# GabeTsai/YOLO-For-Turbines

Measured on AMD Instinct MI355X. Metric: images/sec at 416x416 (fwd), higher is better.
Workload: dtype f32; 1 GPU; BASELINE configs[1]: batch 32/GPU 416x416 fp32 inference, 80-class head, YOLOv3 forward (75 fused conv launches); per_gpu_batch=32, global_batch=32, image_size=416, num_classes=80, parallelism=image-sharded x1 (no collective)

## Files before the change

yolo_for_turbines_amd/csrc/conv_f32_epilogue.h:

```cpp
#pragma once
#include "common.h"

namespace yolo {

typedef float f32x16 __attribute__((ext_vector_type(16)));

struct ConvArgs {
    const float* x;
    const float* w;
    const char* w_planes;
    const float* scale;
    const float* shift;
    const float* res;
    float* y;
    int* nan_flag;
    int N, H, W, Cin, Cout, Ho, Wo, M;
    int ks, stride, pad;
    int x_ld, x_off, y_ld, y_off, r_ld, r_off;
    int Kpad, KT;
    int act, out_mode, flags;
    int nc5;
    int tiles_n;
};

constexpr int BK = 32;

int conv_igemm_launch(const ConvArgs& a, int tile, hipStream_t s);

bool split3_supported(const yolo_conv_desc* d);
bool split3_eligible(const yolo_conv_desc* d);
int conv_split3_launch(const ConvArgs& a, int tile, hipStream_t s);
size_t split3_weight_bytes(const yolo_conv_desc* d);
int split3_weights_launch(const yolo_conv_desc* d, const void* w_packed, void* out, hipStream_t s);

bool splitk_supported(const yolo_conv_desc* d);
bool splitk_eligible(const yolo_conv_desc* d);
int splitk_slices(const yolo_conv_desc* d, int* steps);
size_t splitk_workspace_bytes(const yolo_conv_desc* d);
int conv_splitk_launch(const ConvArgs& a, const yolo_conv_desc* d, void* ws, size_t ws_bytes, hipStream_t s);

__device__ __forceinline__ void conv_f32_store4(const ConvArgs& p, int m, int n, f32x4 v, int HoWo, bool has_res, bool nan_chk, bool& saw_nan) {
    if (has_res) v += *reinterpret_cast<const f32x4*>(p.res + (size_t)m * p.r_ld + p.r_off + n);
    if (nan_chk && (v[0] != v[0] || v[1] != v[1] || v[2] != v[2] || v[3] != v[3])) saw_nan = true;
    if (p.out_mode == YOLO_OUT_NHWC) {
        *reinterpret_cast<f32x4*>(p.y + (size_t)m * p.y_ld + p.y_off + n) = v;
    } else {
        const int img = m / HoWo;
        const int rem = m - img * HoWo;
        const int ho = rem / p.Wo;
        const int wo = rem - ho * p.Wo;
        const int W2 = 2 * p.Wo;
        float* d = p.y + ((size_t)(img * 2 * p.Ho + 2 * ho) * W2 + 2 * wo) * p.y_ld + p.y_off + n;
        *reinterpret_cast<f32x4*>(d) = v;
        *reinterpret_cast<f32x4*>(d + p.y_ld) = v;
        *reinterpret_cast<f32x4*>(d + (size_t)W2 * p.y_ld) = v;
        *reinterpret_cast<f32x4*>(d + (size_t)(W2 + 1) * p.y_ld) = v;
    }
}

__device__ __forceinline__ void conv_f32_store1(const ConvArgs& p, int m, int n, float v, int HoWo, int head_a, int head_k, bool has_res,
                                                bool nan_chk, bool& saw_nan) {
    if (has_res) v += p.res[(size_t)m * p.r_ld + p.r_off + n];
    if (nan_chk && v != v) saw_nan = true;
    if (p.out_mode == YOLO_OUT_NHWC) {
        p.y[(size_t)m * p.y_ld + p.y_off + n] = v;
    } else {
        const int img = m / HoWo;
        const int rem = m - img * HoWo;
        const int ho = rem / p.Wo;
        const int wo = rem - ho * p.Wo;
        if (p.out_mode == YOLO_OUT_UPSAMPLE2X) {
            const int W2 = 2 * p.Wo;
            float* d = p.y + ((size_t)(img * 2 * p.Ho + 2 * ho) * W2 + 2 * wo) * p.y_ld + p.y_off + n;
            d[0] = v;
            d[p.y_ld] = v;
            d[(size_t)W2 * p.y_ld] = v;
            d[(size_t)(W2 + 1) * p.y_ld] = v;
        } else {
            p.y[((size_t)((img * 3 + head_a) * p.Ho + ho) * p.Wo + wo) * p.nc5 + head_k] = v;
        }
    }
}

template <int BM, int BN>
__device__ __forceinline__ void conv_f32_epilogue(const ConvArgs& p, f32x16 (&acc)[BM / 64][BN / 64], float* ost, int m0, int n0) {
    constexpr int WM = BM / 2, WN = BN / 2;
    constexpr int TM = WM / 32, TN = WN / 32;
    const int tid = threadIdx.x;
    const int lane = tid & 63;
    const int wave = tid >> 6;
    const int wm = wave >> 1, wn = wave & 1;
    const int frow = lane & 31, fh = lane >> 5;
    const int HoWo = p.Ho * p.Wo;
    const bool has_res = p.flags & YOLO_FLAG_RESIDUAL;
    const bool nan_chk = p.flags & YOLO_FLAG_NANCHECK;
    bool saw_nan = false;
    const bool aligned4 = ((p.y_ld | p.y_off) & 3) == 0 && (!has_res || ((p.r_ld | p.r_off) & 3) == 0);
    if (p.out_mode != YOLO_OUT_HEAD && (p.Cout & 3) == 0 && aligned4) {
        constexpr int OLD = BN + 4;
#pragma unroll
        for (int j = 0; j < TN; ++j) {
            const int n = n0 + wn * WN + j * 32 + frow;
            const bool nv = n < p.Cout;
            const float sc = nv ? p.scale[n] : 0.f;
            const float sh = nv ? p.shift[n] : 0.f;
            float* dst = ost + wn * WN + j * 32 + frow;
            YOLO_SWITCH_ACT(p.act,
                _Pragma("unroll") for (int i = 0; i < TM; ++i)
                    _Pragma("unroll") for (int r = 0; r < 16; ++r) {
                        const int row = wm * WM + i * 32 + (r & 3) + 8 * (r >> 2) + 4 * fh;
                        dst[row * OLD] = act_c<ACT>(acc[i][j][r] * sc + sh);
                    })
        }
        __syncthreads();
        constexpr int C4 = BN / 4;
#pragma unroll 4
        for (int idx = tid; idx < BM * C4; idx += 256) {
            const int row = idx / C4, c4 = idx - row * C4;
            const int m = m0 + row, n = n0 + c4 * 4;
            if (m >= p.M || n >= p.Cout) continue;
            conv_f32_store4(p, m, n, *reinterpret_cast<const f32x4*>(ost + row * OLD + c4 * 4), HoWo, has_res, nan_chk, saw_nan);
        }
        if (nan_chk && saw_nan) atomicOr(p.nan_flag, 2);
        return;
    }
#pragma unroll
    for (int j = 0; j < TN; ++j) {
        const int n = n0 + wn * WN + j * 32 + frow;
        const bool nv = n < p.Cout;
        const float sc = nv ? p.scale[n] : 0.f;
        const float sh = nv ? p.shift[n] : 0.f;
        int head_a = 0, head_k = 0;
        if (p.out_mode == YOLO_OUT_HEAD) {
            head_a = n / p.nc5;
            head_k = n - head_a * p.nc5;
        }
        YOLO_SWITCH_ACT(p.act,
            _Pragma("unroll") for (int i = 0; i < TM; ++i)
                _Pragma("unroll") for (int r = 0; r < 16; ++r) acc[i][j][r] = act_c<ACT>(acc[i][j][r] * sc + sh);)
#pragma unroll
        for (int i = 0; i < TM; ++i) {
#pragma unroll
            for (int r = 0; r < 16; ++r) {
                const int m = m0 + wm * WM + i * 32 + (r & 3) + 8 * (r >> 2) + 4 * fh;
                if (m >= p.M || !nv) continue;
                conv_f32_store1(p, m, n, acc[i][j][r], HoWo, head_a, head_k, has_res, nan_chk, saw_nan);
            }
        }
    }
    if (nan_chk && saw_nan) atomicOr(p.nan_flag, 2);
}

}
```

yolo_for_turbines_amd/csrc/conv_split3_f32.hip:

```cpp
#include "conv_f32_epilogue.h"
#include "split3.h"

namespace yolo {

constexpr int S3_ROWB = 64;

__device__ __forceinline__ int s3_row_off(int r, int chunk) { return r * S3_ROWB + (((chunk >> 1) ^ ((r >> 2) & 3)) * 16 + (chunk & 1) * 8); }

typedef const __attribute__((address_space(1))) void* s3_gptr;
typedef __attribute__((address_space(3))) void* s3_lptr;
__device__ __forceinline__ void s3_glds16(const void* g, void* l) { __builtin_amdgcn_global_load_lds((s3_gptr)g, (s3_lptr)l, 16, 0, 0); }

struct S3PrepArgs {
    const float* w;
    char* out;
    int Kpad, KT, cp;
};

__global__ __launch_bounds__(256) void split3_weights_f32(const S3PrepArgs p) {
    const int tid = threadIdx.x;
    const int chunk = tid & 7;
    const int n = blockIdx.x * 32 + (tid >> 3);
    const size_t plane_b = (size_t)p.cp * S3_ROWB;
    const float* src = p.w + (size_t)n * p.Kpad + chunk * 4;
    char* dst = p.out + s3_row_off(n, chunk);
    f32x4 chk = {0.f, 0.f, 0.f, 0.f};
    for (int kt = 0; kt < p.KT; ++kt) {
        const f32x4 v = *reinterpret_cast<const f32x4*>(src + kt * BK);
        u32x2 h, m, l;
        s3_split(v, h, m, l, chk);
        char* d = dst + (size_t)kt * 3 * plane_b;
        *reinterpret_cast<u32x2*>(d) = h;
        *reinterpret_cast<u32x2*>(d + plane_b) = m;
        *reinterpret_cast<u32x2*>(d + 2 * plane_b) = l;
    }
    const bool nonfinite = chk[0] != chk[0] || chk[1] != chk[1] || chk[2] != chk[2] || chk[3] != chk[3];
    const int any = __syncthreads_or(nonfinite);
    if (tid == 0) reinterpret_cast<unsigned*>(p.out + (size_t)p.KT * 3 * plane_b)[blockIdx.x] = any ? 1u : 0u;
}

template <int BM, int BN, bool WREADY, bool WDMA>
__global__ __launch_bounds__(256, 2) void conv_split3_f32(const ConvArgs p) {
    static_assert(WREADY || !WDMA, "LDS-DMA needs the prepared weights");
    constexpr int WM = BM / 2, WN = BN / 2;
    constexpr int TM = WM / 32, TN = WN / 32;
    constexpr int RA = BM / 32, RB = BN / 32;
    constexpr bool DBUF = BM + BN <= 128;
    constexpr int A_BYTES = 3 * BM * S3_ROWB;
    constexpr int B_BYTES = 3 * BN * S3_ROWB;
    constexpr int BUF_BYTES = A_BYTES + B_BYTES;
    constexpr bool BRING = DBUF || WDMA;
    constexpr int B_SLOT = DBUF ? BUF_BYTES : B_BYTES;
    constexpr int PB = BN / 64;
    extern __shared__ __attribute__((aligned(16))) char smem_raw[];

    const int tid = threadIdx.x;
    const int lane = tid & 63;
    const int wave = tid >> 6;
    const int wm = wave >> 1, wn = wave & 1;
    const int tile_n = blockIdx.x % p.tiles_n;
    const int tile_m = blockIdx.x / p.tiles_n;
    const int m0 = tile_m * BM, n0 = tile_n * BN;
    const int HoWo = p.Ho * p.Wo;

    auto row_geom = [&](int m, long long& base, unsigned& mask) {
        const bool mv = m < p.M;
        const int mm = mv ? m : 0;
        const int n = mm / HoWo;
        const int rem = mm - n * HoWo;
        const int ho = rem / p.Wo;
        const int wo = rem - ho * p.Wo;
        const int hi0 = ho * p.stride - p.pad, wi0 = wo * p.stride - p.pad;
        base = ((long long)(n * p.H + hi0) * p.W + wi0) * p.x_ld + p.x_off;
        unsigned mk = 0;
        for (int kh = 0; kh < p.ks; ++kh)
            for (int kw = 0; kw < p.ks; ++kw)
                if (mv && (unsigned)(hi0 + kh) < (unsigned)p.H && (unsigned)(wi0 + kw) < (unsigned)p.W)
                    mk |= 1u << (kh * p.ks + kw);
        mask = mk;
    };

    const int chunk = tid & 7;
    const int lrow = tid >> 3;
    long long a_base[RA];
    unsigned a_mask[RA];
#pragma unroll
    for (int i = 0; i < RA; ++i) row_geom(m0 + lrow + 32 * i, a_base[i], a_mask[i]);
    const float* wrow = p.w + (size_t)(n0 + lrow) * p.Kpad + chunk * 4;
    const char* wq = p.w_planes;
    const size_t plane_b = (size_t)((p.Cout + 127) & ~127) * S3_ROWB;
    const char* wsrc = wq + (size_t)n0 * S3_ROWB + tid * 16;

    f32x4 ra[RA], rb[RB];
    s3_u32x4 rw[3][PB];
    f32x4 chk = {0.f, 0.f, 0.f, 0.f};
    auto load_global = [&](int kt) {
        const int kg = kt * BK;
        const int tap = kg / p.Cin;
        const int coff = kg - tap * p.Cin + chunk * 4;
        const int kh = tap / p.ks, kw = tap - kh * p.ks;
        const long long toff = (long long)(kh * p.W + kw) * p.x_ld + coff;
#pragma unroll
        for (int i = 0; i < RA; ++i) {
            const bool v = (a_mask[i] >> tap) & 1u;
            f32x4 z = {0.f, 0.f, 0.f, 0.f};
            ra[i] = v ? *reinterpret_cast<const f32x4*>(p.x + a_base[i] + toff) : z;
        }
        if constexpr (!WREADY) {
#pragma unroll
            for (int i = 0; i < RB; ++i)
                rb[i] = *reinterpret_cast<const f32x4*>(wrow + (size_t)(32 * i) * p.Kpad + kt * BK);
        } else {
            const char* src = wsrc + (size_t)kt * 3 * plane_b;
            char* dst = smem_raw + A_BYTES + (kt & 1) * B_SLOT + wave * 1024;
#pragma unroll
            for (int q = 0; q < 3; ++q)
#pragma unroll
                for (int i = 0; i < PB; ++i) {
                    if constexpr (WDMA)
                        s3_glds16(src + q * plane_b + i * 4096, dst + q * BN * S3_ROWB + i * 4096);
                    else
                        rw[q][i] = *reinterpret_cast<const s3_u32x4*>(src + q * plane_b + i * 4096);
                }
        }
    };
    auto store_lds = [&](int buf, int bslot) {
        char* a = smem_raw + buf * BUF_BYTES + s3_row_off(lrow, chunk);
        char* b = smem_raw + A_BYTES + bslot * B_SLOT + s3_row_off(lrow, chunk);
#pragma unroll
        for (int i = 0; i < RA; ++i) {
            u32x2 h, m, l;
            s3_split(ra[i], h, m, l, chk);
            *reinterpret_cast<u32x2*>(a + (0 * BM + 32 * i) * S3_ROWB) = h;
            *reinterpret_cast<u32x2*>(a + (1 * BM + 32 * i) * S3_ROWB) = m;
            *reinterpret_cast<u32x2*>(a + (2 * BM + 32 * i) * S3_ROWB) = l;
        }
        if constexpr (!WREADY) {
#pragma unroll
            for (int i = 0; i < RB; ++i) {
                u32x2 h, m, l;
                s3_split(rb[i], h, m, l, chk);
                *reinterpret_cast<u32x2*>(b + (0 * BN + 32 * i) * S3_ROWB) = h;
                *reinterpret_cast<u32x2*>(b + (1 * BN + 32 * i) * S3_ROWB) = m;
                *reinterpret_cast<u32x2*>(b + (2 * BN + 32 * i) * S3_ROWB) = l;
            }
        } else if constexpr (!WDMA) {
            char* bw = smem_raw + A_BYTES + bslot * B_SLOT + tid * 16;
#pragma unroll
            for (int q = 0; q < 3; ++q)
#pragma unroll
                for (int i = 0; i < PB; ++i) *reinterpret_cast<s3_u32x4*>(bw + q * BN * S3_ROWB + i * 4096) = rw[q][i];
        }
    };

    f32x16 acc[TM][TN];
#pragma unroll
    for (int i = 0; i < TM; ++i)
#pragma unroll
        for (int j = 0; j < TN; ++j)
#pragma unroll
            for (int r = 0; r < 16; ++r) acc[i][j][r] = 0.f;

    const int frow = lane & 31, fh = lane >> 5;
    const int a_frag = (wm * WM + frow) * S3_ROWB;
    const int b_frag = A_BYTES + (wn * WN + frow) * S3_ROWB;
    const int fsw = (frow >> 2) & 3;
    const int f_slot[2] = {(fh ^ fsw) * 16, ((2 + fh) ^ fsw) * 16};

    load_global(0);
    store_lds(0, 0);
    if constexpr (WDMA) asm volatile("s_waitcnt vmcnt(0)" ::: "memory");
    __syncthreads();

    for (int kt = 0; kt < p.KT; ++kt) {
        const int cur = DBUF ? (kt & 1) : 0;
        const int bcur = BRING ? (kt & 1) : 0;
        const bool more = kt + 1 < p.KT;
        if (more) load_global(kt + 1);
        const char* Ab = smem_raw + cur * BUF_BYTES + a_frag;
        const char* Bb = smem_raw + bcur * B_SLOT + b_frag;
#pragma unroll
        for (int c = 0; c < 2; ++c) {
            s3_bf16x8 af[TM][3], bf[TN][3];
#pragma unroll
            for (int i = 0; i < TM; ++i)
#pragma unroll
                for (int q = 0; q < 3; ++q)
                    af[i][q] = *reinterpret_cast<const s3_bf16x8*>(Ab + (q * BM + i * 32) * S3_ROWB + f_slot[c]);
#pragma unroll
            for (int j = 0; j < TN; ++j)
#pragma unroll
                for (int q = 0; q < 3; ++q)
                    bf[j][q] = *reinterpret_cast<const s3_bf16x8*>(Bb + (q * BN + j * 32) * S3_ROWB + f_slot[c]);
            constexpr int QA[6] = {0, 2, 1, 0, 1, 0};
            constexpr int QB[6] = {2, 0, 1, 1, 0, 0};
#pragma unroll
            for (int t = 0; t < 6; ++t)
#pragma unroll
                for (int i = 0; i < TM; ++i)
#pragma unroll
                    for (int j = 0; j < TN; ++j)
                        acc[i][j] = __builtin_amdgcn_mfma_f32_32x32x16_bf16(af[i][QA[t]], bf[j][QB[t]], acc[i][j], 0, 0, 0);
        }
        if (!DBUF) __syncthreads();
        if (more) store_lds(DBUF ? (cur ^ 1) : 0, BRING ? (bcur ^ 1) : 0);
        if constexpr (WDMA) asm volatile("s_waitcnt vmcnt(0)" ::: "memory");
        __syncthreads();
    }

    bool nonfinite = chk[0] != chk[0] || chk[1] != chk[1] || chk[2] != chk[2] || chk[3] != chk[3];
    if constexpr (WREADY) {
        const unsigned* table = reinterpret_cast<const unsigned*>(wq + (size_t)p.KT * 3 * plane_b);
#pragma unroll
        for (int g = 0; g < BN / 32; ++g) nonfinite |= table[n0 / 32 + g] != 0;
    }
    if (__syncthreads_or(nonfinite)) {
        long long f_base[TM];
        unsigned f_mask[TM];
#pragma unroll
        for (int i = 0; i < TM; ++i) row_geom(m0 + wm * WM + i * 32 + frow, f_base[i], f_mask[i]);
        const float* fw = p.w + (size_t)(n0 + wn * WN + frow) * p.Kpad + 4 * fh;
#pragma unroll
        for (int i = 0; i < TM; ++i)
#pragma unroll
            for (int j = 0; j < TN; ++j)
#pragma unroll
                for (int r = 0; r < 16; ++r) acc[i][j][r] = 0.f;
        for (int kt = 0; kt < p.KT; ++kt) {
            const int kg = kt * BK;
            const int tap = kg / p.Cin;
            const int kh = tap / p.ks, kw = tap - kh * p.ks;
            const long long toff = (long long)(kh * p.W + kw) * p.x_ld + (kg - tap * p.Cin) + 4 * fh;
            for (int s = 0; s < 4; ++s) {
                f32x4 af[TM], bf[TN];
#pragma unroll
                for (int i = 0; i < TM; ++i) {
                    f32x4 z = {0.f, 0.f, 0.f, 0.f};
                    af[i] = ((f_mask[i] >> tap) & 1u) ? *reinterpret_cast<const f32x4*>(p.x + f_base[i] + toff + s * 8) : z;
                }
#pragma unroll
                for (int j = 0; j < TN; ++j) bf[j] = *reinterpret_cast<const f32x4*>(fw + (size_t)(32 * j) * p.Kpad + kg + s * 8);
#pragma unroll
                for (int e = 0; e < 4; ++e)
#pragma unroll
                    for (int i = 0; i < TM; ++i)
#pragma unroll
                        for (int j = 0; j < TN; ++j)
                            acc[i][j] = __builtin_amdgcn_mfma_f32_32x32x2f32(af[i][e], bf[j][e], acc[i][j], 0, 0, 0);
            }
        }
    }

    conv_f32_epilogue<BM, BN>(p, acc, reinterpret_cast<float*>(smem_raw), m0, n0);
}

bool split3_supported(const yolo_conv_desc* d) {
    return d->dtype == YOLO_F32 && (d->ksize == 1 || d->ksize == 3) && (d->stride == 1 || d->stride == 2) && d->cin % 32 == 0;
}

template <int BM, int BN, bool WREADY, bool WDMA>
static int launch_split3(const ConvArgs& a, hipStream_t s) {
    constexpr bool dbuf = BM + BN <= 128;
    constexpr size_t operands = dbuf ? (size_t)2 * 3 * (BM + BN) * S3_ROWB : (size_t)3 * (BM + (WDMA ? 2 : 1) * BN) * S3_ROWB;
    constexpr size_t transpose = (size_t)BM * (BN + 4) * sizeof(float);
    constexpr size_t lds = operands > transpose ? operands : transpose;
    ConvArgs p = a;
    p.tiles_n = ceil_div(a.Cout, BN);
    const long long blocks = (long long)ceil_div(a.M, BM) * p.tiles_n;
    if (blocks > 0x7fffffffLL) return fail(YOLO_ERR_UNSUPPORTED, "conv_split3_f32: too many blocks");
    if (lds > 64 * 1024) {
        static LdsOnce once;
        if (int rc = reserve_lds(once, reinterpret_cast<const void*>(&conv_split3_f32<BM, BN, WREADY, WDMA>), lds, "conv_split3_f32")) return rc;
    }
    hipLaunchKernelGGL((conv_split3_f32<BM, BN, WREADY, WDMA>), dim3((unsigned)blocks), dim3(256), lds, s, p);
    return check_launch("conv_split3_f32");
}

constexpr bool kS3Dma128x128 = true, kS3Dma128x64 = false, kS3Dma64x64 = true;

template <int BM, int BN, bool WDMA>
static int launch_split3(const ConvArgs& a, hipStream_t s) {
    return a.w_planes ? launch_split3<BM, BN, true, WDMA>(a, s) : launch_split3<BM, BN, false, false>(a, s);
}

size_t split3_weight_bytes(const yolo_conv_desc* d) {
    const size_t cp = coutpad_of(d->cout), KT = kpad_of(d->cin, d->ksize) / BK;
    return packed_f32(d->cout, d->cin, d->ksize).tail_bytes + KT * 3 * cp * S3_ROWB + cp / 32 * sizeof(unsigned);
}

int split3_weights_launch(const yolo_conv_desc* d, const void* w_packed, void* out, hipStream_t s) {
    const size_t off = packed_f32(d->cout, d->cin, d->ksize).tail_bytes;
    if (out != w_packed) {
        const char *a = static_cast<const char*>(w_packed), *b = static_cast<const char*>(out);
        if (a < b + split3_weight_bytes(d) && b < a + off) return fail(YOLO_ERR_ARG, "yolo_split3_weights: out overlaps w_packed (pass the same pointer to prepare in place)");
        if (hipMemcpyAsync(out, w_packed, off, hipMemcpyDeviceToDevice, s) != hipSuccess) return check_launch("yolo_split3_weights: copy");
    }
    S3PrepArgs p;
    p.w = static_cast<const float*>(w_packed);
    p.out = static_cast<char*>(out) + off;
    p.Kpad = kpad_of(d->cin, d->ksize);
    p.KT = p.Kpad / BK;
    p.cp = coutpad_of(d->cout);
    hipLaunchKernelGGL(split3_weights_f32, dim3(p.cp / 32), dim3(256), 0, s, p);
    return check_launch("split3_weights_f32");
}

static int pick_split3_tile(const ConvArgs& a, bool ready) {
    if (a.ks == 3 && a.stride == 2 && a.Cin >= 64 && (ready || a.Cin < 512)) return kTileF32Reg128x128;
    if (a.ks == 1 && (long long)a.H * a.W * a.Cout < 100000) return kTileF32Reg64x64;
    if (ready && a.ks == 1 && a.Cout % 128 == 0 && a.Cin >= ((long long)a.H * a.W >= 52 * 52 ? 256 : 768)) return kTileF32Reg128x128;
    return kTileF32Reg128x64;
}

bool split3_eligible(const yolo_conv_desc* d) {
    if (!split3_supported(d)) return false;
    if (d->ksize == 3) return d->stride == 2 || (d->cin == 32 && (long long)d->h * d->w >= 208 * 208);
    return d->stride == 1 && (long long)d->h * d->w * d->cout >= 40000;
}

int conv_split3_launch(const ConvArgs& a, int tile, hipStream_t s) {
    switch (tile ? tile : pick_split3_tile(a, a.w_planes != nullptr)) {
    case kTileF32Reg128x128: return launch_split3<128, 128, kS3Dma128x128>(a, s);
    case kTileF32Reg128x64: return launch_split3<128, 64, kS3Dma128x64>(a, s);
    case kTileF32Reg64x64: return launch_split3<64, 64, kS3Dma64x64>(a, s);
    default: return fail(YOLO_ERR_UNSUPPORTED, "conv: YOLO_FLAG_SPLIT_BF16 has tiles 1 (128x128), 2 (128x64) and 4 (64x64), not %d", tile);
    }
}

}
```

Baseline: 3064 images/s.

## Add DMA-fed double-buffered split3 kernel for 128x128 tiles with 4x1 wave layout

Adds a new conv_split3d_f32 kernel, used for 128x128 split3 tiles when prepared weight planes exist. It loads both the im2col activation rows and the bf16 weight planes straight into LDS through global_load_lds, double-buffered across K steps. Each wave owns 32 rows across the full N width, so the epilogue is generalised to a 4x1 wave grid. The aim is to cut VGPR staging and improve load/compute overlap, at the cost of different LDS traffic and occupancy, and it relies on a zero line in global memory for padded taps.

```diff
diff --git a/yolo_for_turbines_amd/csrc/conv_f32_epilogue.h b/yolo_for_turbines_amd/csrc/conv_f32_epilogue.h
--- a/yolo_for_turbines_amd/csrc/conv_f32_epilogue.h
+++ b/yolo_for_turbines_amd/csrc/conv_f32_epilogue.h
@@ -82,14 +82,15 @@
     }
 }
 
-template <int BM, int BN>
-__device__ __forceinline__ void conv_f32_epilogue(const ConvArgs& p, f32x16 (&acc)[BM / 64][BN / 64], float* ost, int m0, int n0) {
-    constexpr int WM = BM / 2, WN = BN / 2;
+template <int BM, int BN, int WGM = 2>
+__device__ __forceinline__ void conv_f32_epilogue(const ConvArgs& p, f32x16 (&acc)[BM / (32 * WGM)][BN * WGM / 128], float* ost, int m0, int n0) {
+    constexpr int WGN = 4 / WGM;
+    constexpr int WM = BM / WGM, WN = BN / WGN;
     constexpr int TM = WM / 32, TN = WN / 32;
     const int tid = threadIdx.x;
     const int lane = tid & 63;
     const int wave = tid >> 6;
-    const int wm = wave >> 1, wn = wave & 1;
+    const int wm = wave / WGN, wn = wave % WGN;
     const int frow = lane & 31, fh = lane >> 5;
     const int HoWo = p.Ho * p.Wo;
     const bool has_res = p.flags & YOLO_FLAG_RESIDUAL;
diff --git a/yolo_for_turbines_amd/csrc/conv_split3.h b/yolo_for_turbines_amd/csrc/conv_split3.h
--- /dev/null
+++ b/yolo_for_turbines_amd/csrc/conv_split3.h
@@ -0,0 +1,72 @@
+#pragma once
+#include "conv_f32_epilogue.h"
+#include "split3.h"
+
+namespace yolo {
+
+constexpr int S3_ROWB = 64;
+
+typedef const __attribute__((address_space(1))) void* s3_gptr;
+typedef __attribute__((address_space(3))) void* s3_lptr;
+__device__ __forceinline__ void s3_glds16(const void* g, void* l) { __builtin_amdgcn_global_load_lds((s3_gptr)g, (s3_lptr)l, 16, 0, 0); }
+
+__device__ __forceinline__ void s3_row_geom(const ConvArgs& p, int HoWo, int m, long long& base, unsigned& mask) {
+    const bool mv = m < p.M;
+    const int mm = mv ? m : 0;
+    const int n = mm / HoWo;
+    const int rem = mm - n * HoWo;
+    const int ho = rem / p.Wo;
+    const int wo = rem - ho * p.Wo;
+    const int hi0 = ho * p.stride - p.pad, wi0 = wo * p.stride - p.pad;
+    base = ((long long)(n * p.H + hi0) * p.W + wi0) * p.x_ld + p.x_off;
+    unsigned mk = 0;
+    for (int kh = 0; kh < p.ks; ++kh)
+        for (int kw = 0; kw < p.ks; ++kw)
+            if (mv && (unsigned)(hi0 + kh) < (unsigned)p.H && (unsigned)(wi0 + kw) < (unsigned)p.W)
+                mk |= 1u << (kh * p.ks + kw);
+    mask = mk;
+}
+
+template <int TM, int TN>
+__device__ __forceinline__ void s3_exact_tile(const ConvArgs& p, f32x16 (&acc)[TM][TN], int mw, int nw, int HoWo) {
+    const int lane = threadIdx.x & 63;
+    const int frow = lane & 31, fh = lane >> 5;
+    long long f_base[TM];
+    unsigned f_mask[TM];
+#pragma unroll
+    for (int i = 0; i < TM; ++i) s3_row_geom(p, HoWo, mw + i * 32 + frow, f_base[i], f_mask[i]);
+    const float* fw = p.w + (size_t)(nw + frow) * p.Kpad + 4 * fh;
+#pragma unroll
+    for (int i = 0; i < TM; ++i)
+#pragma unroll
+        for (int j = 0; j < TN; ++j)
+#pragma unroll
+            for (int r = 0; r < 16; ++r) acc[i][j][r] = 0.f;
+    for (int kt = 0; kt < p.KT; ++kt) {
+        const int kg = kt * BK;
+        const int tap = kg / p.Cin;
+        const int kh = tap / p.ks, kw = tap - kh * p.ks;
+        const long long toff = (long long)(kh * p.W + kw) * p.x_ld + (kg - tap * p.Cin) + 4 * fh;
+        for (int s = 0; s < 4; ++s) {
+            f32x4 af[TM], bf[TN];
+#pragma unroll
+            for (int i = 0; i < TM; ++i) {
+                f32x4 z = {0.f, 0.f, 0.f, 0.f};
+                af[i] = ((f_mask[i] >> tap) & 1u) ? *reinterpret_cast<const f32x4*>(p.x + f_base[i] + toff + s * 8) : z;
+            }
+#pragma unroll
+            for (int j = 0; j < TN; ++j) bf[j] = *reinterpret_cast<const f32x4*>(fw + (size_t)(32 * j) * p.Kpad + kg + s * 8);
+#pragma unroll
+            for (int e = 0; e < 4; ++e)
+#pragma unroll
+                for (int i = 0; i < TM; ++i)
+#pragma unroll
+                    for (int j = 0; j < TN; ++j)
+                        acc[i][j] = __builtin_amdgcn_mfma_f32_32x32x2f32(af[i][e], bf[j][e], acc[i][j], 0, 0, 0);
+        }
+    }
+}
+
+int conv_split3d_launch(const ConvArgs& a, hipStream_t s);
+
+}
diff --git a/yolo_for_turbines_amd/csrc/conv_split3_f32.hip b/yolo_for_turbines_amd/csrc/conv_split3_f32.hip
--- a/yolo_for_turbines_amd/csrc/conv_split3_f32.hip
+++ b/yolo_for_turbines_amd/csrc/conv_split3_f32.hip
@@ -1,15 +1,8 @@
-#include "conv_f32_epilogue.h"
-#include "split3.h"
+#include "conv_split3.h"
 
 namespace yolo {
 
-constexpr int S3_ROWB = 64;
-
 __device__ __forceinline__ int s3_row_off(int r, int chunk) { return r * S3_ROWB + (((chunk >> 1) ^ ((r >> 2) & 3)) * 16 + (chunk & 1) * 8); }
-
-typedef const __attribute__((address_space(1))) void* s3_gptr;
-typedef __attribute__((address_space(3))) void* s3_lptr;
-__device__ __forceinline__ void s3_glds16(const void* g, void* l) { __builtin_amdgcn_global_load_lds((s3_gptr)g, (s3_lptr)l, 16, 0, 0); }
 
 struct S3PrepArgs {
     const float* w;
@@ -63,29 +56,12 @@
     const int m0 = tile_m * BM, n0 = tile_n * BN;
     const int HoWo = p.Ho * p.Wo;
 
-    auto row_geom = [&](int m, long long& base, unsigned& mask) {
-        const bool mv = m < p.M;
-        const int mm = mv ? m : 0;
-        const int n = mm / HoWo;
-        const int rem = mm - n * HoWo;
-        const int ho = rem / p.Wo;
-        const int wo = rem - ho * p.Wo;
-        const int hi0 = ho * p.stride - p.pad, wi0 = wo * p.stride - p.pad;
-        base = ((long long)(n * p.H + hi0) * p.W + wi0) * p.x_ld + p.x_off;
-        unsigned mk = 0;
-        for (int kh = 0; kh < p.ks; ++kh)
-            for (int kw = 0; kw < p.ks; ++kw)
-                if (mv && (unsigned)(hi0 + kh) < (unsigned)p.H && (unsigned)(wi0 + kw) < (unsigned)p.W)
-                    mk |= 1u << (kh * p.ks + kw);
-        mask = mk;
-    };
-
     const int chunk = tid & 7;
     const int lrow = tid >> 3;
     long long a_base[RA];
     unsigned a_mask[RA];
 #pragma unroll
-    for (int i = 0; i < RA; ++i) row_geom(m0 + lrow + 32 * i, a_base[i], a_mask[i]);
+    for (int i = 0; i < RA; ++i) s3_row_geom(p, HoWo, m0 + lrow + 32 * i, a_base[i], a_mask[i]);
     const float* wrow = p.w + (size_t)(n0 + lrow) * p.Kpad + chunk * 4;
     const char* wq = p.w_planes;
     const size_t plane_b = (size_t)((p.Cout + 127) & ~127) * S3_ROWB;
@@ -214,42 +190,7 @@
 #pragma unroll
         for (int g = 0; g < BN / 32; ++g) nonfinite |= table[n0 / 32 + g] != 0;
     }
-    if (__syncthreads_or(nonfinite)) {
-        long long f_base[TM];
-        unsigned f_mask[TM];
-#pragma unroll
-        for (int i = 0; i < TM; ++i) row_geom(m0 + wm * WM + i * 32 + frow, f_base[i], f_mask[i]);
-        const float* fw = p.w + (size_t)(n0 + wn * WN + frow) * p.Kpad + 4 * fh;
-#pragma unroll
-        for (int i = 0; i < TM; ++i)
-#pragma unroll
-            for (int j = 0; j < TN; ++j)
-#pragma unroll
-                for (int r = 0; r < 16; ++r) acc[i][j][r] = 0.f;
-        for (int kt = 0; kt < p.KT; ++kt) {
-            const int kg = kt * BK;
-            const int tap = kg / p.Cin;
-            const int kh = tap / p.ks, kw = tap - kh * p.ks;
-            const long long toff = (long long)(kh * p.W + kw) * p.x_ld + (kg - tap * p.Cin) + 4 * fh;
-            for (int s = 0; s < 4; ++s) {
-                f32x4 af[TM], bf[TN];
-#pragma unroll
-                for (int i = 0; i < TM; ++i) {
-                    f32x4 z = {0.f, 0.f, 0.f, 0.f};
-                    af[i] = ((f_mask[i] >> tap) & 1u) ? *reinterpret_cast<const f32x4*>(p.x + f_base[i] + toff + s * 8) : z;
-                }
-#pragma unroll
-                for (int j = 0; j < TN; ++j) bf[j] = *reinterpret_cast<const f32x4*>(fw + (size_t)(32 * j) * p.Kpad + kg + s * 8);
-#pragma unroll
-                for (int e = 0; e < 4; ++e)
-#pragma unroll
-                    for (int i = 0; i < TM; ++i)
-#pragma unroll
-                        for (int j = 0; j < TN; ++j)
-                            acc[i][j] = __builtin_amdgcn_mfma_f32_32x32x2f32(af[i][e], bf[j][e], acc[i][j], 0, 0, 0);
-            }
-        }
-    }
+    if (__syncthreads_or(nonfinite)) s3_exact_tile<TM, TN>(p, acc, m0 + wm * WM, n0 + wn * WN, HoWo);
 
     conv_f32_epilogue<BM, BN>(p, acc, reinterpret_cast<float*>(smem_raw), m0, n0);
 }
@@ -276,11 +217,18 @@
     return check_launch("conv_split3_f32");
 }
 
-constexpr bool kS3Dma128x128 = true, kS3Dma128x64 = false, kS3Dma64x64 = true;
-
-template <int BM, int BN, bool WDMA>
+enum S3Ready { kS3Regs, kS3DmaB, kS3DmaAB };
+constexpr S3Ready kS3Ready128x128 = kS3DmaAB, kS3Ready128x64 = kS3Regs, kS3Ready64x64 = kS3DmaB;
+
+template <int BM, int BN, S3Ready READY>
 static int launch_split3(const ConvArgs& a, hipStream_t s) {
-    return a.w_planes ? launch_split3<BM, BN, true, WDMA>(a, s) : launch_split3<BM, BN, false, false>(a, s);
+    if (!a.w_planes) return launch_split3<BM, BN, false, false>(a, s);
+    if constexpr (READY == kS3DmaAB) {
+        static_assert(BM == 128 && BN == 128, "conv_split3d_f32 has 128x128 blocks");
+        return conv_split3d_launch(a, s);
+    } else {
+        return launch_split3<BM, BN, true, READY == kS3DmaB>(a, s);
+    }
 }
 
 size_t split3_weight_bytes(const yolo_conv_desc* d) {
@@ -320,9 +268,9 @@
 
 int conv_split3_launch(const ConvArgs& a, int tile, hipStream_t s) {
     switch (tile ? tile : pick_split3_tile(a, a.w_planes != nullptr)) {
-    case kTileF32Reg128x128: return launch_split3<128, 128, kS3Dma128x128>(a, s);
-    case kTileF32Reg128x64: return launch_split3<128, 64, kS3Dma128x64>(a, s);
-    case kTileF32Reg64x64: return launch_split3<64, 64, kS3Dma64x64>(a, s);
+    case kTileF32Reg128x128: return launch_split3<128, 128, kS3Ready128x128>(a, s);
+    case kTileF32Reg128x64: return launch_split3<128, 64, kS3Ready128x64>(a, s);
+    case kTileF32Reg64x64: return launch_split3<64, 64, kS3Ready64x64>(a, s);
     default: return fail(YOLO_ERR_UNSUPPORTED, "conv: YOLO_FLAG_SPLIT_BF16 has tiles 1 (128x128), 2 (128x64) and 4 (64x64), not %d", tile);
     }
 }
diff --git a/yolo_for_turbines_amd/csrc/conv_split3d_f32.hip b/yolo_for_turbines_amd/csrc/conv_split3d_f32.hip
--- /dev/null
+++ b/yolo_for_turbines_amd/csrc/conv_split3d_f32.hip
@@ -0,0 +1,163 @@
+#include "conv_split3.h"
+
+namespace yolo {
+
+static __device__ __attribute__((aligned(128))) unsigned int g_s3_zero_line[32];
+
+constexpr int S3D_BM = 128;
+constexpr int S3D_LINE = 128;
+
+template <int BN>
+__global__ __launch_bounds__(256, 2) void conv_split3d_f32(const ConvArgs p) {
+    constexpr int BM = S3D_BM;
+    constexpr int TN = BN / 32;
+    constexpr int A_BYTES = BM * S3D_LINE;
+    constexpr int B_BYTES = 3 * BN * S3_ROWB;
+    constexpr int SLOT = A_BYTES + B_BYTES;
+    constexpr int PB = BN / 64;
+    extern __shared__ __attribute__((aligned(16))) char smem_raw[];
+
+    const int tid = threadIdx.x;
+    const int lane = tid & 63;
+    const int wave = tid >> 6;
+    const int tile_n = blockIdx.x % p.tiles_n;
+    const int tile_m = blockIdx.x / p.tiles_n;
+    const int m0 = tile_m * BM, n0 = tile_n * BN;
+    const int HoWo = p.Ho * p.Wo;
+
+    const float* a_src[4];
+    unsigned a_mask[4];
+#pragma unroll
+    for (int i = 0; i < 4; ++i) {
+        long long base;
+        s3_row_geom(p, HoWo, m0 + 32 * wave + 8 * i + (lane >> 3), base, a_mask[i]);
+        a_src[i] = p.x + base + 4 * ((lane & 7) ^ ((4 * i + (lane >> 4)) & 7));
+    }
+    const float* zline = reinterpret_cast<const float*>(g_s3_zero_line) + 4 * (lane & 7);
+    const size_t plane_b = (size_t)((p.Cout + 127) & ~127) * S3_ROWB;
+    const char* wsrc = p.w_planes + (size_t)n0 * S3_ROWB + tid * 16;
+
+    int r_tap = 0, r_kh = 0, r_kw = 0, r_c = 0;
+    auto request = [&](int kt, int slot) {
+        char* dst = smem_raw + slot * SLOT;
+        const long long toff = (long long)(r_kh * p.W + r_kw) * p.x_ld + r_c;
+#pragma unroll
+        for (int i = 0; i < 4; ++i)
+            s3_glds16(((a_mask[i] >> r_tap) & 1u) ? a_src[i] + toff : zline, dst + (32 * wave + 8 * i) * S3D_LINE);
+        const char* src = wsrc + (size_t)kt * 3 * plane_b;
+#pragma unroll
+        for (int q = 0; q < 3; ++q)
+#pragma unroll
+            for (int i = 0; i < PB; ++i)
+                s3_glds16(src + q * plane_b + i * 4096, dst + A_BYTES + wave * 1024 + q * BN * S3_ROWB + i * 4096);
+        r_c += BK;
+        if (r_c == p.Cin) {
+            r_c = 0;
+            ++r_tap;
+            if (++r_kw == p.ks) { r_kw = 0; ++r_kh; }
+        }
+    };
+
+    f32x16 acc[1][TN];
+#pragma unroll
+    for (int j = 0; j < TN; ++j)
+#pragma unroll
+        for (int r = 0; r < 16; ++r) acc[0][j][r] = 0.f;
+
+    const int frow = lane & 31, fh = lane >> 5;
+    const int fa = (frow >> 1) & 7;
+    const int a_frag = (32 * wave + frow) * S3D_LINE;
+    const int a_off[2][2] = {{a_frag + ((2 * fh) ^ fa) * 16, a_frag + ((2 * fh + 1) ^ fa) * 16},
+                             {a_frag + ((4 + 2 * fh) ^ fa) * 16, a_frag + ((5 + 2 * fh) ^ fa) * 16}};
+    const int fsw = (frow >> 2) & 3;
+    const int b_frag = A_BYTES + frow * S3_ROWB;
+    const int b_off[2] = {b_frag + (fh ^ fsw) * 16, b_frag + ((2 + fh) ^ fsw) * 16};
+
+    f32x4 chk = {0.f, 0.f, 0.f, 0.f};
+    auto read_a = [&](const char* S, int c, f32x4 (&r)[2]) {
+        r[0] = *reinterpret_cast<const f32x4*>(S + a_off[c][0]);
+        r[1] = *reinterpret_cast<const f32x4*>(S + a_off[c][1]);
+    };
+    auto read_b = [&](const char* S, int c, s3_bf16x8 (&b)[TN][3]) {
+#pragma unroll
+        for (int q = 0; q < 3; ++q)
+#pragma unroll
+            for (int j = 0; j < TN; ++j) b[j][q] = *reinterpret_cast<const s3_bf16x8*>(S + (q * BN + j * 32) * S3_ROWB + b_off[c]);
+    };
+    auto split_a = [&](const f32x4 (&r)[2], s3_bf16x8 (&a)[3]) {
+        u32x2 h0, m0_, l0, h1, m1, l1;
+        s3_split(r[0], h0, m0_, l0, chk);
+        s3_split(r[1], h1, m1, l1, chk);
+        a[0] = __builtin_bit_cast(s3_bf16x8, s3_u32x4{h0[0], h0[1], h1[0], h1[1]});
+        a[1] = __builtin_bit_cast(s3_bf16x8, s3_u32x4{m0_[0], m0_[1], m1[0], m1[1]});
+        a[2] = __builtin_bit_cast(s3_bf16x8, s3_u32x4{l0[0], l0[1], l1[0], l1[1]});
+    };
+    auto mma = [&](const s3_bf16x8 (&a)[3], const s3_bf16x8 (&b)[TN][3]) {
+        constexpr int QA[6] = {0, 2, 1, 0, 1, 0};
+        constexpr int QB[6] = {2, 0, 1, 1, 0, 0};
+#pragma unroll
+        for (int t = 0; t < 6; ++t)
+#pragma unroll
+            for (int j = 0; j < TN; ++j)
+                acc[0][j] = __builtin_amdgcn_mfma_f32_32x32x16_bf16(a[QA[t]], b[j][QB[t]], acc[0][j], 0, 0, 0);
+    };
+
+    request(0, 0);
+    asm volatile("s_waitcnt vmcnt(0)" ::: "memory");
+    __syncthreads();
+
+    for (int kt = 0; kt < p.KT; ++kt) {
+        const int cur = kt & 1;
+        if (kt + 1 < p.KT) request(kt + 1, cur ^ 1);
+        const char* S = smem_raw + cur * SLOT;
+        f32x4 ra0[2], ra1[2];
+        s3_bf16x8 af[3], b0[TN][3], b1[TN][3];
+        read_a(S, 0, ra0);
+        read_b(S, 0, b0);
+        read_a(S, 1, ra1);
+        read_b(S, 1, b1);
+        split_a(ra0, af);
+        mma(af, b0);
+        split_a(ra1, af);
+        mma(af, b1);
+        asm volatile("s_waitcnt vmcnt(0)" ::: "memory");
+        __syncthreads();
+    }
+
+    bool nonfinite = chk[0] != chk[0] || chk[1] != chk[1] || chk[2] != chk[2] || chk[3] != chk[3];
+    {
+        const unsigned* table = reinterpret_cast<const unsigned*>(p.w_planes + (size_t)p.KT * 3 * plane_b);
+#pragma unroll
+        for (int g = 0; g < BN / 32; ++g) nonfinite |= table[n0 / 32 + g] != 0;
+    }
+    unsigned* vote = reinterpret_cast<unsigned*>(smem_raw);
+    const bool wave_nonfinite = __ballot(nonfinite) != 0;
+    if (lane == 0) vote[wave] = wave_nonfinite;
+    __syncthreads();
+    const bool exact = (vote[0] | vote[1] | vote[2] | vote[3]) != 0;
+    __syncthreads();
+    if (exact) s3_exact_tile<1, TN>(p, acc, m0 + 32 * wave, n0, HoWo);
+
+    conv_f32_epilogue<BM, BN, 4>(p, acc, reinterpret_cast<float*>(smem_raw), m0, n0);
+}
+
+template <int BN>
+static int launch_split3d(const ConvArgs& a, hipStream_t s) {
+    constexpr size_t ring = (size_t)2 * (S3D_BM * S3D_LINE + 3 * BN * S3_ROWB);
+    constexpr size_t transpose = (size_t)S3D_BM * (BN + 4) * sizeof(float);
+    constexpr size_t lds = ring > transpose ? ring : transpose;
+    ConvArgs p = a;
+    p.tiles_n = ceil_div(a.Cout, BN);
+    const long long blocks = (long long)ceil_div(a.M, S3D_BM) * p.tiles_n;
+    if (blocks > 0x7fffffffLL) return fail(YOLO_ERR_UNSUPPORTED, "conv_split3_f32: too many blocks");
+    if (lds > 64 * 1024) {
+        static LdsOnce once;
+        if (int rc = reserve_lds(once, reinterpret_cast<const void*>(&conv_split3d_f32<BN>), lds, "conv_split3_f32")) return rc;
+    }
+    hipLaunchKernelGGL((conv_split3d_f32<BN>), dim3((unsigned)blocks), dim3(256), lds, s, p);
+    return check_launch("conv_split3_f32");
+}
+
+int conv_split3d_launch(const ConvArgs& a, hipStream_t s) { return launch_split3d<128>(a, s); }
+
+}
```

Result: no change. 3049 images/s (-0.5%).
